# paultsw/wavenet-speech

Hardware: AMD Instinct MI355X
Metric: samples/sec fwd+bwd, 256-ch 30-block WaveNet @16k seq (higher is better)
Workload: dtype f32; 1 GPU; BASELINE.json configs[2]: WaveNet 256 ch, 30 blocks (3 x dilation 1..512), k=2, seq_len 16000, batch 16 per GPU, f32, full step (fwd+bwd+grad all-reduce+Adam); channels=256, blocks=30, seq_len=16000, batch_per_gpu=16, global_batch=16, parallelism=dp1, params=16037632, input=dense one-hot, init=reference

## Files before the change

wavenet_speech_amd/csrc/wn_api.hip:

```cpp
#include <hip/hip_runtime.h>

#include <algorithm>
#include <cstdio>
#include <cstdlib>
#include <cstdint>
#include <cstring>
#include <mutex>
#include <string>
#include <vector>

#include "../../include/wavenet_amd.h"
#include "wn_kernels.h"

using namespace wn;

#ifdef WN_STAMPS
namespace wn { extern int g_debug_kc; }
#endif

namespace {

thread_local std::string g_hip_err;

int hip_fail(hipError_t e, const char* what) {
// ... 204 lines not shown
    for (int i = 0; i < g.nslab; ++i) {
        a.slab_woff[i] = g.slab_woff[i];
        a.slab_nseg[i] = g.slab_nseg[i];
        a.slab_boff[i] = g.slab_boff[i];
    }
    a.wpacked = reinterpret_cast<float*>((char*)packed + off);
    a.bias = reinterpret_cast<float*>((char*)packed + off + align256((size_t)g.wfloats * 4));
    a.total = g.wfloats;
}

void fill_gemm_common(GemmArgs& a, const GemmPlan& g, const void* packed, size_t off, int first_slab, int nslab,
                      int B, int L, int ld, int halo) {
    std::memset(&a, 0, sizeof(a));
    a.wpacked = plan_w(packed, off);
    a.bias = plan_b(packed, off, g);
    a.nslab = nslab;
    for (int i = 0; i < nslab; ++i) {
        GemmSlab& s = a.slab[i];
        s.woff = g.slab_woff[first_slab + i];
        s.nseg = g.slab_nseg[first_slab + i];
        s.dst = g.slab_dst[first_slab + i];
        s.row0 = g.slab_row0[first_slab + i];
        s.boff = g.slab_boff[first_slab + i];
    }
    a.B = B; a.L = L; a.ld = ld; a.halo = halo;
    a.tiles_per_row = cdiv(L, kColTile);
    a.ncol = B * a.tiles_per_row;
}

inline void set_seg(GemmArgs& a, int i, const float* base, int c, int off, int nkb) {
    a.seg[i].base = base; a.seg[i].cp = cp8(c); a.seg[i].off = off; a.seg[i].nkb = nkb;
}

inline PackSrc mk_src(const float* p, int rows, int cols, int sr, int sc) {
    PackSrc s; s.ptr = p; s.rows = rows; s.cols = cols; s.stride_r = sr; s.stride_c = sc; return s;
}

struct WgradPlan {
    int WT = 1, npair = 0, ntile_total = 0, nsplit = 1;
    int Mp[kMaxPair], Np[kMaxPair], mt[kMaxPair], nt[kMaxPair], tile0[kMaxPair], rs_off[kMaxPair];
    long long slab_off[kMaxPair];
    long long slab_floats = 0;
    int rs_floats = 0;
    void add(int M, int N) {
        const int T = 64 * WT, i = npair++;
        mt[i] = cdiv(M, T); nt[i] = cdiv(N, T);
        Mp[i] = mt[i] * T; Np[i] = nt[i] * T;
        tile0[i] = ntile_total; ntile_total += mt[i] * nt[i];
        slab_off[i] = slab_floats; slab_floats += (long long)Mp[i] * Np[i];
        rs_off[i] = rs_floats; rs_floats += Mp[i];
    }
    void finish(int nchunk) {
        nsplit = std::max(1, 512 / std::max(1, ntile_total));
        nsplit = std::min(nsplit, std::max(1, nchunk));
        if (nsplit >= 16) nsplit = nsplit / 8 * 8;
    }
    bool xcd_map() const { return nsplit % 8 == 0; }
    size_t bytes() const { return (size_t)nsplit * (size_t)(slab_floats + rs_floats) * 4; }
};
inline int pick_wt(int maxdim) { return maxdim > 128 ? 4 : (maxdim > 64 ? 2 : 1); }

}


int wn_version(void) { return WN_VERSION; }

// ... 19 lines not shown
}

int wn_tap_offsets(int k, int d, int causal, int* off) {
    if (!off) return WN_ERR_NULL;
    if (k < 1 || d < 1) return WN_ERR_BAD_SHAPE;
    return tap_offsets(k, d, causal, off);
}

int wn_series_layout(int length, int max_abs_offset, int* ld, int* halo) {
    if (!ld || !halo) return WN_ERR_NULL;
    if (length <= 0 || max_abs_offset < 0) return WN_ERR_BAD_SHAPE;
    *halo = rup(max_abs_offset, 4);
    *ld = 2 * (*halo) + rup(length, kColTile);
    return WN_OK;
}

size_t wn_series_floats(int batch, int channels, int ld) { return (size_t)batch * cp8(channels) * (size_t)ld; }

size_t wn_block_packed_bytes(const wn_block_shape* s) {
    int off[WN_MAX_TAPS];
    if (check_block(s, off) != WN_OK) return 0;
    return plan_block(s).total;
}

int wn_block_pack(const wn_block_shape* s, const wn_block_params* p, void* packed, wn_stream_t stream) {
    int off[WN_MAX_TAPS];
    int rc = check_block(s, off);
    if (rc != WN_OK) return rc;
    if (!p || !packed || !p->w_tanh || !p->w_sigmoid || !p->w_res || !p->w_skip || !p->w_proj) return WN_ERR_NULL;
    hipStream_t st = (hipStream_t)stream;
    const BlockPlan bp = plan_block(s);
    const int Ci = s->in_channels, Co = s->out_channels, Ms = s->skip_rows, k = s->kernel_width;
    ProfScope prof(KC_PACK, 0.0, st);
    PackArgs a;
    {
        const GemmPlan& g = bp.fa;
        fill_pack_common(a, g, packed, bp.off_fa);
        for (int j = 0; j < k; ++j) {
            a.set[0].seg[j] = mk_src(p->w_tanh + j, Co, Ci, Ci * k, k);
            a.set[1].seg[j] = mk_src(p->w_sigmoid + j, Co, Ci, Ci * k, k);
        }
        a.set[0].bias0 = p->b_tanh; a.set[0].bias_rows = Co;
        a.set[1].bias0 = p->b_sigmoid; a.set[1].bias_rows = Co;
        const int pairs = tiles32(Co);
        for (int sl = 0; sl < g.nslab; ++sl)
            for (int m = 0; m < g.MT; ++m) {
                const int pair = sl * (g.MT / 2) + m / 2;
                a.tile[sl * g.MT + m].set = m & 1;
                a.tile[sl * g.MT + m].row0 = pair < pairs ? 32 * pair : -1;
            }
        WN_HIP(launch_pack(a, st), "pack(gate)");
    }
    {
        const GemmPlan& g = bp.fb;
        fill_pack_common(a, g, packed, bp.off_fb);
        a.set[0].seg[0] = mk_src(p->w_res, Co, Co, Co, 1);
        a.set[0].seg[1] = mk_src(p->w_proj, Co, Ci, Ci, 1);
        a.set[0].bias0 = p->b_res; a.set[0].bias1 = p->b_proj; a.set[0].bias_rows = Co;
        a.set[1].seg[0] = mk_src(p->w_skip, Ms, Co, Co, 1);
        a.set[1].bias0 = p->b_skip; a.set[1].bias_rows = Ms;
        for (int sl = 0; sl < g.nslab; ++sl)
            for (int m = 0; m < g.MT; ++m) {
                const bool skip = sl >= bp.fb_first_skip_slab;
                const int row0 = g.slab_row0[sl] + 32 * m;
                a.tile[sl * g.MT + m].set = skip ? 1 : 0;
                a.tile[sl * g.MT + m].row0 = row0 < (skip ? Ms : Co) ? row0 : -1;
            }
        WN_HIP(launch_pack(a, st), "pack(res+skip)");
    }
    {
        const GemmPlan& g = bp.ka;
        fill_pack_common(a, g, packed, bp.off_ka);
        a.set[0].seg[0] = mk_src(p->w_skip, Co, Ms, 1, Co);
        a.set[0].seg[1] = mk_src(p->w_res, Co, Co, 1, Co);
        for (int sl = 0; sl < g.nslab; ++sl)
            for (int m = 0; m < g.MT; ++m) {
                const int row0 = g.slab_row0[sl] + 32 * m;
                a.tile[sl * g.MT + m].set = 0;
                a.tile[sl * g.MT + m].row0 = row0 < Co ? row0 : -1;
            }
        WN_HIP(launch_pack(a, st), "pack(dz)");
    }
    {
        const GemmPlan& g = bp.kb;
        fill_pack_common(a, g, packed, bp.off_kb);
        for (int j = 0; j < k; ++j) {
            a.set[0].seg[2 * j] = mk_src(p->w_tanh + j, Ci, Co, k, Ci * k);
            a.set[0].seg[2 * j + 1] = mk_src(p->w_sigmoid + j, Ci, Co, k, Ci * k);
        }
        a.set[0].seg[2 * k] = mk_src(p->w_proj, Ci, Co, 1, Ci);
        for (int sl = 0; sl < g.nslab; ++sl)
            for (int m = 0; m < g.MT; ++m) {
                const int row0 = g.slab_row0[sl] + 32 * m;
                a.tile[sl * g.MT + m].set = 0;
                a.tile[sl * g.MT + m].row0 = row0 < Ci ? row0 : -1;
            }
        WN_HIP(launch_pack(a, st), "pack(dx)");
    }
    return WN_OK;
}

int wn_block_forward(const wn_block_shape* s, const void* packed, const float* x, float* r_out, float* skip,
                     int skip_accumulate, float* sg, float* z, wn_stream_t stream) {
    int off[WN_MAX_TAPS];
    int rc = check_block(s, off);
    if (rc != WN_OK) return rc;
    if (!packed || !x || !z) return WN_ERR_NULL;
    hipStream_t st = (hipStream_t)stream;
    const BlockPlan bp = plan_block(s);
    const int Ci = s->in_channels, Co = s->out_channels, Ms = s->skip_rows, k = s->kernel_width;
    const double BL = (double)s->batch * s->length;
    GemmArgs a;
    {
        const GemmPlan& g = bp.fa;
        fill_gemm_common(a, g, packed, bp.off_fa, 0, g.nslab, s->batch, s->length, s->ld, s->halo);
        for (int j = 0; j < k; ++j) set_seg(a, j, x, Ci, off[j], g.seg_nkb[j]);
        a.sg = sg; a.z = z; a.gate_cp = cp8(Co); a.gate_rows = Co;
        ProfScope prof(KC_GATE_GEMM, 2.0 * (2.0 * Co) * (double)(k * Ci) * BL, st);
        WN_HIP(launch_gemm(g.MT, EPI_GATE, a, st), "series_gemm<gate>");
    }
    {
        const GemmPlan& g = bp.fb;
        const double fl_r = 2.0 * Co * (double)(Co + Ci) * BL, fl_s = 2.0 * Ms * (double)Co * BL;
        if (r_out) {
            fill_gemm_common(a, g, packed, bp.off_fb, 0, bp.fb_first_skip_slab, s->batch, s->length, s->ld, s->halo);
            set_seg(a, 0, z, Co, 0, g.seg_nkb[0]);
            set_seg(a, 1, x, Ci, 0, g.seg_nkb[1]);
            a.dst[0].base = r_out; a.dst[0].cp = cp8(Co); a.dst[0].rows = Co; a.dst[0].accumulate = 0;
            ProfScope prof(KC_OUT_GEMM, fl_r, st);
            WN_HIP(launch_gemm(g.MT, EPI_LINEAR, a, st), "series_gemm<res>");
        }
// ... 67 lines not shown
    const int t = tiles32(s->skip_rows);
    g.MT = pick_mt(t);
    g.nseg = s->nblocks;
    for (int l = 0; l < s->nblocks; ++l) g.seg_nkb[l] = cp8(s->channels[l]) / 8;
    for (int i = 0; i < cdiv(t, g.MT); ++i) g.add_slab(s->nblocks, i * g.MT * 32, 0);
    return g;
}
}

size_t wn_skipsum_packed_bytes(const wn_skipsum_shape* s) {
    if (check_skipsum(s) != WN_OK) return 0;
    return plan_skipsum(s).bytes();
}

int wn_skipsum_pack(const wn_skipsum_shape* s, const float* const* w_skip, const float* bias_total, void* packed,
                    wn_stream_t stream) {
    int rc = check_skipsum(s);
    if (rc != WN_OK) return rc;
    if (!w_skip || !packed) return WN_ERR_NULL;
    for (int l = 0; l < s->nblocks; ++l) if (!w_skip[l]) return WN_ERR_NULL;
    hipStream_t st = (hipStream_t)stream;
    const GemmPlan g = plan_skipsum(s);
    ProfScope prof(KC_PACK, 0.0, st);
    PackArgs a;
    fill_pack_common(a, g, packed, 0);
    for (int l = 0; l < s->nblocks; ++l) a.set[0].seg[l] = mk_src(w_skip[l], s->skip_rows, s->channels[l], s->channels[l], 1);
    a.set[0].bias0 = bias_total; a.set[0].bias_rows = s->skip_rows;
    for (int sl = 0; sl < g.nslab; ++sl)
        for (int m = 0; m < g.MT; ++m) {
            const int row0 = g.slab_row0[sl] + 32 * m;
            a.tile[sl * g.MT + m].set = 0;
            a.tile[sl * g.MT + m].row0 = row0 < s->skip_rows ? row0 : -1;
        }
    WN_HIP(launch_pack(a, st), "pack(skipsum)");
    return WN_OK;
}

int wn_skipsum_forward(const wn_skipsum_shape* s, const void* packed, const float* const* z, float* skip, int accumulate,
                       wn_stream_t stream) {
    int rc = check_skipsum(s);
    if (rc != WN_OK) return rc;
    if (!packed || !z || !skip) return WN_ERR_NULL;
    for (int l = 0; l < s->nblocks; ++l) if (!z[l]) return WN_ERR_NULL;
    hipStream_t st = (hipStream_t)stream;
    const GemmPlan g = plan_skipsum(s);
    GemmArgs a;
    fill_gemm_common(a, g, packed, 0, 0, g.nslab, s->batch, s->length, s->ld, s->halo);
    double ksum = 0;
    for (int l = 0; l < s->nblocks; ++l) { set_seg(a, l, z[l], s->channels[l], 0, g.seg_nkb[l]); ksum += s->channels[l]; }
    a.dst[0].base = skip; a.dst[0].cp = cp8(s->skip_rows); a.dst[0].rows = s->skip_rows; a.dst[0].accumulate = accumulate ? 1 : 0;
    ProfScope prof(KC_SKIP_GEMM, 2.0 * s->skip_rows * ksum * (double)s->batch * s->length, st);
    WN_HIP(launch_gemm(g.MT, accumulate ? EPI_ACCUM : EPI_LINEAR, a, st), "series_gemm<skipsum>");
    return WN_OK;
}

namespace {
struct PairSpec { const float* A; int a_rows; const float* Bm; int b_rows; int off; int rowsum;
                  float* w; int sm, sn; float* b0; float* b1; };

int run_wgrad(const std::vector<PairSpec>& ps, int maxdim, int B, int L, int ld, int halo, void* workspace,
              size_t workspace_bytes, bool dry, size_t* need, int kc, hipStream_t st) {
    WgradPlan wp;
    wp.WT = pick_wt(maxdim);
    for (const PairSpec& p : ps) wp.add(p.a_rows, p.b_rows);
    const int cpr = cdiv(L, 32);
    wp.finish(B * cpr);
    if (need) *need = wp.bytes();
// ... 114 lines not shown
        GemmPlan& g = p.cf;
        const int t = tiles32(Co);
        g.MT = pick_mt(t); g.nseg = k;
        for (int j = 0; j < k; ++j) g.seg_nkb[j] = cp8(Ci) / 8;
        for (int i = 0; i < cdiv(t, g.MT); ++i) g.add_slab(k, i * g.MT * 32, 0);
    }
    {
        GemmPlan& g = p.cb;
        const int t = tiles32(Ci);
        g.MT = pick_mt(t); g.nseg = k;
        for (int j = 0; j < k; ++j) g.seg_nkb[j] = cp8(Co) / 8;
        for (int i = 0; i < cdiv(t, g.MT); ++i) g.add_slab(k, i * g.MT * 32, 0);
    }
    p.off_cf = 0; p.off_cb = p.cf.bytes(); p.total = p.off_cb + p.cb.bytes();
    return p;
}
}

size_t wn_conv_packed_bytes(const wn_conv_shape* s) {
    int off[WN_MAX_TAPS];
    if (check_conv(s, off) != WN_OK) return 0;
    return plan_conv(s).total;
}

int wn_conv_pack(const wn_conv_shape* s, const float* weight, const float* bias, void* packed, wn_stream_t stream) {
    int off[WN_MAX_TAPS];
    int rc = check_conv(s, off);
    if (rc != WN_OK) return rc;
    if (!weight || !packed) return WN_ERR_NULL;
    hipStream_t st = (hipStream_t)stream;
    const ConvPlan cp = plan_conv(s);
    const int Ci = s->in_channels, Co = s->out_channels, k = s->kernel_width;
    ProfScope prof(KC_PACK, 0.0, st);
    PackArgs a;
    {
        const GemmPlan& g = cp.cf;
        fill_pack_common(a, g, packed, cp.off_cf);
        for (int j = 0; j < k; ++j) a.set[0].seg[j] = mk_src(weight + j, Co, Ci, Ci * k, k);
        a.set[0].bias0 = bias; a.set[0].bias_rows = Co;
        for (int sl = 0; sl < g.nslab; ++sl)
            for (int m = 0; m < g.MT; ++m) {
                const int row0 = g.slab_row0[sl] + 32 * m;
                a.tile[sl * g.MT + m].set = 0;
                a.tile[sl * g.MT + m].row0 = row0 < Co ? row0 : -1;
            }
        WN_HIP(launch_pack(a, st), "pack(conv fwd)");
    }
    {
        const GemmPlan& g = cp.cb;
        fill_pack_common(a, g, packed, cp.off_cb);
        for (int j = 0; j < k; ++j) a.set[0].seg[j] = mk_src(weight + j, Ci, Co, k, Ci * k);
        for (int sl = 0; sl < g.nslab; ++sl)
            for (int m = 0; m < g.MT; ++m) {
                const int row0 = g.slab_row0[sl] + 32 * m;
                a.tile[sl * g.MT + m].set = 0;
                a.tile[sl * g.MT + m].row0 = row0 < Ci ? row0 : -1;
            }
        WN_HIP(launch_pack(a, st), "pack(conv bwd)");
    }
    return WN_OK;
}

int wn_conv_forward(const wn_conv_shape* s, const void* packed, const float* x, float* y, wn_stream_t stream) {
    int off[WN_MAX_TAPS];
    int rc = check_conv(s, off);
    if (rc != WN_OK) return rc;
    if (!packed || !x || !y) return WN_ERR_NULL;
    hipStream_t st = (hipStream_t)stream;
    const ConvPlan cp = plan_conv(s);
    const GemmPlan& g = cp.cf;
    GemmArgs a;
    fill_gemm_common(a, g, packed, cp.off_cf, 0, g.nslab, s->batch, s->length, s->ld, s->halo);
    for (int j = 0; j < s->kernel_width; ++j) set_seg(a, j, x, s->in_channels, off[j], g.seg_nkb[j]);
    a.dst[0].base = y; a.dst[0].cp = cp8(s->out_channels); a.dst[0].rows = s->out_channels; a.dst[0].accumulate = 0;
    ProfScope prof(KC_CONV_FWD, 2.0 * s->out_channels * (double)(s->kernel_width * s->in_channels) * s->batch * s->length, st);
    WN_HIP(launch_gemm(g.MT, EPI_LINEAR, a, st), "series_gemm<conv fwd>");
    return WN_OK;
}

int wn_conv_backward_data(const wn_conv_shape* s, const void* packed, const float* dy, float* dx, wn_stream_t stream) {
    int off[WN_MAX_TAPS];
    int rc = check_conv(s, off);
    if (rc != WN_OK) return rc;
    if (!packed || !dy || !dx) return WN_ERR_NULL;
    hipStream_t st = (hipStream_t)stream;
    const ConvPlan cp = plan_conv(s);
    const GemmPlan& g = cp.cb;
    GemmArgs a;
    fill_gemm_common(a, g, packed, cp.off_cb, 0, g.nslab, s->batch, s->length, s->ld, s->halo);
    a.bias = nullptr;
    for (int j = 0; j < s->kernel_width; ++j) set_seg(a, j, dy, s->out_channels, -off[j], g.seg_nkb[j]);
    a.dst[0].base = dx; a.dst[0].cp = cp8(s->in_channels); a.dst[0].rows = s->in_channels; a.dst[0].accumulate = 0;
// ... 98 lines not shown
```

wavenet_speech_amd/csrc/wn_gemm.hip:

```cpp
#include <cstdlib>

#include "wn_kernels.h"

namespace wn {

__device__ __forceinline__ int rowof(int r, int h) { return (r & 3) + 8 * (r >> 2) + 4 * h; }

__device__ __forceinline__ float sigmoid_f(float x) {
    const float e = __builtin_amdgcn_exp2f(-1.44269504088896341f * x);
    return __builtin_amdgcn_rcpf(1.0f + e);
}
__device__ __forceinline__ float tanh_f(float x) {
    const float ax = __builtin_fabsf(x);
    const float e = __builtin_amdgcn_exp2f(-2.88539008177792681f * ax);
    const float big = (1.0f - e) * __builtin_amdgcn_rcpf(1.0f + e);
    const float x2 = x * x;
    const float small = ax * (1.0f + x2 * (-0.333333333f + x2 * (0.133333333f + x2 * -0.0539682540f)));
    return __builtin_copysignf(ax < 0.125f ? small : big, x);
}

template <int NT> struct BVec;
template <> struct BVec<4> { typedef f32x4 reg_t; };
template <> struct BVec<2> { typedef float __attribute__((ext_vector_type(2))) reg_t; };

template <int MT, int NT, int EPI, int PFB, int WPS>
__global__ __launch_bounds__(64, WPS) void series_gemm_kernel(const GemmArgs a) {
    typedef typename BVec<NT>::reg_t breg_t;
    constexpr int COLS = 32 * NT;
    const int lane = threadIdx.x;
    const int n0 = lane & 31, h0 = lane >> 5;
#ifdef WN_STAMPS
    const unsigned long long st_t0 = __builtin_amdgcn_s_memtime(), st_r0 = __builtin_amdgcn_s_memrealtime();
    unsigned long long st_t1 = 0, st_t2 = 0;
#endif

    const int id = blockIdx.x;
    const int xcd = id & 7, local = id >> 3;
    const int slab_i = local % a.nslab;
    const int coltile = (local / a.nslab) * 8 + xcd;
    if (coltile >= a.ncol) return;
    const int b = coltile / a.tiles_per_row;
    const int t0 = (coltile - b * a.tiles_per_row) * COLS;
    const GemmSlab sl = a.slab[slab_i];
    const int ld = a.ld;

    f32x16 acc[MT][NT];
    const float* bias_p = (a.bias ? a.bias : a.wpacked) + sl.boff;
    const float bias_on = a.bias ? 1.0f : 0.0f;
#pragma unroll
    for (int m = 0; m < MT; ++m) {
#pragma unroll
        for (int r = 0; r < 16; ++r) {
            const float bv = bias_p[32 * m + rowof(r, h0)] * bias_on;
#pragma unroll
            for (int t = 0; t < NT; ++t) acc[m][t][r] = bv;
        }
    }

    int nkb = 0;
    for (int s = 0; s < sl.nseg; ++s) nkb += a.seg[s].nkb;

    constexpr unsigned kRsrcFlags = 0x00020000u;
    auto resource = [&](const float* base) {
        return __builtin_amdgcn_make_buffer_rsrc(const_cast<float*>(base), 0, 0xffffffffu, kRsrcFlags);
    };
    const __amdgpu_buffer_rsrc_t wrs = resource(a.wpacked + sl.woff);
    const unsigned a_off = lane * 16u;
    unsigned a_soff = 0;
    const long tilebase = (long)a.halo + t0;
    unsigned b_off[4];
#pragma unroll
    for (int q = 0; q < 4; ++q) b_off[q] = 4u * ((unsigned)(4 * h0 + q) * (unsigned)ld + (unsigned)(NT * n0));
    int seg = 0;
    int seg_left = a.seg[0].nkb;
    __amdgpu_buffer_rsrc_t brs = resource(a.seg[0].base + (long)b * a.seg[0].cp * ld);
    unsigned b_soff = 4u * (unsigned)(tilebase + a.seg[0].off);
    int b_left = nkb;
    const unsigned a_last = (unsigned)(nkb > 0 ? nkb - 1 : 0) * (MT * 1024u);

    f32x4 A[2][MT];
    breg_t B[4][4];
// ... 36 lines not shown
    for (int p = 0; p < PFB; ++p) loadB(B[p]);
#ifdef WN_STAMPS
    __builtin_amdgcn_sched_barrier(0);
    st_t1 = __builtin_amdgcn_s_memtime();
    __builtin_amdgcn_sched_barrier(0);
#endif
    int g0 = 0;
    for (; g0 + 4 <= nkb; g0 += 4) {
#pragma unroll
        for (int j = 0; j < 4; ++j) {
            loadA(A[(j + 1) & 1]);
            loadB(B[(j + PFB) & 3]);
            __builtin_amdgcn_sched_barrier(0);
            compute(A[j & 1], B[j & 3]);
            __builtin_amdgcn_sched_barrier(0);
        }
    }
#pragma unroll
    for (int j = 0; j < 3; ++j) {
        if (g0 + j < nkb) {
            loadA(A[(j + 1) & 1]);
            loadB(B[(j + PFB) & 3]);
            __builtin_amdgcn_sched_barrier(0);
            compute(A[j & 1], B[j & 3]);
            __builtin_amdgcn_sched_barrier(0);
        }
    }

#ifdef WN_STAMPS
    __builtin_amdgcn_sched_barrier(0);
    st_t2 = __builtin_amdgcn_s_memtime();
    __builtin_amdgcn_sched_barrier(0);
    struct StampOut {
        unsigned long long* p; unsigned long long t0, r0, t1, t2; int lane;
        __device__ ~StampOut() {
            __builtin_amdgcn_sched_barrier(0);
            const unsigned long long t_issued = __builtin_amdgcn_s_memtime();
            __builtin_amdgcn_sched_barrier(0);
            asm volatile("s_waitcnt vmcnt(0)" ::: "memory");
            if (p && lane == 0) {
                p[0] = t0; p[1] = t1; p[2] = t2; p[3] = __builtin_amdgcn_s_memtime();
                p[4] = r0; p[5] = __builtin_amdgcn_s_memrealtime();
                p[6] = __builtin_amdgcn_s_getreg(63492);
                p[7] = (unsigned long long)__builtin_amdgcn_s_getreg(63508) | ((t_issued - t2) << 32);
            }
        }
    } stamp_out{a.stamps ? a.stamps + 8ull * blockIdx.x : nullptr, st_t0, st_r0, st_t1, st_t2, lane};
#endif
    const int lane_e = (int)__builtin_amdgcn_mbcnt_hi(~0u, __builtin_amdgcn_mbcnt_lo(~0u, 0u));
    const int n = lane_e & 31, h = lane_e >> 5;
    const long colbase = tilebase + NT * n;
    const int c0 = t0 + NT * n;
    if (c0 >= a.L) return;
    auto clip = [&](breg_t v) {
#pragma unroll
        for (int t = 1; t < NT; ++t)
            if (c0 + t >= a.L) v[t] = 0.0f;
        return v;
    };

    if constexpr (EPI == EPI_LINEAR) {
        const GemmDst d = a.dst[sl.dst];
#pragma unroll
        for (int m = 0; m < MT; ++m) {
#pragma unroll
            for (int r = 0; r < 16; ++r) {
                const int row = sl.row0 + 32 * m + rowof(r, h);
                if (row < d.rows) {
                    float* p = d.base + ((long)b * d.cp + row) * ld + colbase;
                    breg_t v;
#pragma unroll
                    for (int t = 0; t < NT; ++t) v[t] = acc[m][t][r];
                    *reinterpret_cast<breg_t*>(p) = clip(v);
                }
            }
            __builtin_amdgcn_sched_barrier(0);
        }
    } else if constexpr (EPI == EPI_ACCUM) {
        const GemmDst d = a.dst[sl.dst];
        constexpr int RB = 8, BPT = 16 / RB, NBATCH = MT * BPT;
        breg_t old[2][RB];
        float* const tile = d.base + (long)b * d.cp * ld + colbase;
        auto fetch = [&](int bi, breg_t (&dst)[RB]) {
            const int m = bi / BPT, r0 = (bi % BPT) * RB;
#pragma unroll
            for (int i = 0; i < RB; ++i) {
                int row = sl.row0 + 32 * m + rowof(r0 + i, h);
                row = row < d.rows ? row : d.rows - 1;
                dst[i] = *reinterpret_cast<const breg_t*>(tile + (long)row * ld);
            }
        };
        fetch(0, old[0]);
#pragma unroll
        for (int bi = 0; bi < NBATCH; ++bi) {
            if (bi + 1 < NBATCH) fetch(bi + 1, old[(bi + 1) & 1]);
            __builtin_amdgcn_sched_barrier(0);
            const int m = bi / BPT, r0 = (bi % BPT) * RB;
#pragma unroll
            for (int i = 0; i < RB; ++i) {
                const int row = sl.row0 + 32 * m + rowof(r0 + i, h);
                if (row < d.rows) {
                    breg_t v;
#pragma unroll
                    for (int t = 0; t < NT; ++t) v[t] = acc[m][t][r0 + i] + old[bi & 1][i][t];
                    *reinterpret_cast<breg_t*>(tile + (long)row * ld) = clip(v);
                }
            }
            __builtin_amdgcn_sched_barrier(0);
        }
    } else if constexpr (EPI == EPI_GATE) {
#pragma unroll
        for (int i = 0; i < MT / 2; ++i) {
#pragma unroll
            for (int r = 0; r < 16; ++r) {
                const int ch = sl.row0 + 32 * i + rowof(r, h);
                if (ch < a.gate_rows) {
                    breg_t vs, vz;
#pragma unroll
                    for (int t = 0; t < NT; ++t) {
                        const float tt = tanh_f(acc[2 * i][t][r]);
                        const float ss = sigmoid_f(acc[2 * i + 1][t][r]);
                        vs[t] = ss;
                        vz[t] = tt * ss;
                    }
                    const long o = ((long)b * a.gate_cp + ch) * ld + colbase;
                    *reinterpret_cast<breg_t*>(a.z + o) = clip(vz);
                    if (a.sg) *reinterpret_cast<breg_t*>(a.sg + o) = clip(vs);
                }
            }
            __builtin_amdgcn_sched_barrier(0);
        }
    } else {
        constexpr int RB = (MT == 4) ? 8 : 4;
        constexpr int BPT = 16 / RB;
        constexpr int NBATCH = MT * BPT;
        breg_t vt[2][RB], vs[2][RB];
        auto fetch = [&](int bi, breg_t (&ft)[RB], breg_t (&fs)[RB]) {
            const int m = bi / BPT, r0 = (bi % BPT) * RB;
#pragma unroll
            for (int i = 0; i < RB; ++i) {
                int ch = sl.row0 + 32 * m + rowof(r0 + i, h);
                ch = ch < a.gate_rows ? ch : a.gate_rows - 1;
                const long o = ((long)b * a.gate_cp + ch) * ld + colbase;
                ft[i] = *reinterpret_cast<const breg_t*>(a.z + o);
                fs[i] = *reinterpret_cast<const breg_t*>(a.sg + o);
            }
        };
        fetch(0, vt[0], vs[0]);
#pragma unroll
        for (int bi = 0; bi < NBATCH; ++bi) {
            if (bi + 1 < NBATCH) fetch(bi + 1, vt[(bi + 1) & 1], vs[(bi + 1) & 1]);
            __builtin_amdgcn_sched_barrier(0);
            const int m = bi / BPT, r0 = (bi % BPT) * RB;
#pragma unroll
            for (int i = 0; i < RB; ++i) {
                const int r = r0 + i;
                const int ch = sl.row0 + 32 * m + rowof(r, h);
                if (ch < a.gate_rows) {
                    const long o = ((long)b * a.gate_cp + ch) * ld + colbase;
                    const breg_t z_ = vt[bi & 1][i], sg_ = vs[bi & 1][i];
                    breg_t va, vg;
#pragma unroll
                    for (int t = 0; t < NT; ++t) {
                        const float dz = acc[m][t][r];
                        const float tt = sg_[t] > 0.0f ? z_[t] / sg_[t] : 0.0f;
                        va[t] = dz * (sg_[t] - z_[t] * tt);
                        vg[t] = dz * z_[t] * (1.0f - sg_[t]);
                    }
                    *reinterpret_cast<breg_t*>(a.da + o) = clip(va);
                    *reinterpret_cast<breg_t*>(a.dg + o) = clip(vg);
                }
            }
            __builtin_amdgcn_sched_barrier(0);
        }
    }
}

#ifdef WN_STAMPS
static unsigned long long* g_stamp_buf = nullptr;
static int g_stamp_kc = -1;
int g_debug_kc = -1;
extern "C" void wn_debug_set_stamp_buffer(void* p) { g_stamp_buf = (unsigned long long*)p; }
extern "C" void wn_debug_set_stamp_class(int kc) { g_stamp_kc = kc; }
extern "C" unsigned wn_debug_last_grid = 0;
#endif

template <int MT, int NT, int EPI, int PFB, int WPS>
static hipError_t launch_one(GemmArgs a, hipStream_t st) {
#ifdef WN_STAMPS
    const bool stamp_this = g_stamp_buf && (g_stamp_kc < 0 || g_stamp_kc == g_debug_kc);
    a.stamps = stamp_this ? g_stamp_buf : nullptr;
#endif
    a.tiles_per_row = (a.L + 32 * NT - 1) / (32 * NT);
    a.ncol = a.B * a.tiles_per_row;
    const int ncol8 = (a.ncol + 7) / 8 * 8;
    const unsigned grid = (unsigned)(a.nslab * ncol8);
#ifdef WN_STAMPS
    if (stamp_this) wn_debug_last_grid = grid;
#endif
    hipLaunchKernelGGL((series_gemm_kernel<MT, NT, EPI, PFB, WPS>), dim3(grid), dim3(64), 0, st, a);
    return hipGetLastError();
}

static int gemm_variant() {
    static int v = -1;
    if (v < 0) {
        const char* e = getenv("WN_GEMM_VARIANT");
        v = e ? atoi(e) : 0;
    }
    return v;
}

template <int EPI>
static hipError_t launch_epi(int MT, const GemmArgs& a, hipStream_t st) {
    const int v = gemm_variant();
    if (MT == 4) {
        if (v == 1) return launch_one<4, 4, EPI, 1, 1>(a, st);
        return launch_one<4, 4, EPI, 3, 1>(a, st);
    }
    if (MT == 2) return launch_one<2, 4, EPI, 3, 2>(a, st);
    if constexpr (EPI != EPI_GATE) {
        if (MT == 1) return launch_one<1, 4, EPI, 3, 2>(a, st);
    }
    return hipErrorInvalidValue;
}

hipError_t launch_gemm(int MT, int epi, const GemmArgs& a, hipStream_t st) {
    if (a.nslab <= 0 || a.B <= 0 || a.L <= 0) return hipSuccess;
    switch (epi) {
        case EPI_LINEAR: return launch_epi<EPI_LINEAR>(MT, a, st);
        case EPI_GATE: return launch_epi<EPI_GATE>(MT, a, st);
// ... 8 lines not shown
```

wavenet_speech_amd/csrc/wn_kernels.h:

```cpp
#pragma once
#include <hip/hip_runtime.h>
#include <stdint.h>

namespace wn {

typedef float f32x16 __attribute__((ext_vector_type(16)));
typedef float f32x4 __attribute__((ext_vector_type(4)));

constexpr int kMaxSeg = 32;
constexpr int kMaxSlab = 32;
constexpr int kMaxDst = 2;
constexpr int kColTile = 128;

struct GemmSeg {
    const float* base;
    int cp;
    int off;
    int nkb;
    int _pad;
};

struct GemmSlab {
    long long woff;
    int nseg;
// ... 27 lines not shown
    int tiles_per_row;
    int ncol;
    unsigned long long* stamps;
};

enum { EPI_LINEAR = 0, EPI_GATE = 1, EPI_DGATE = 2, EPI_ACCUM = 3 };

struct PackSrc {
    const float* ptr;
    int rows, cols;
    int stride_r, stride_c;
};
struct PackSet {
    PackSrc seg[kMaxSeg];
    const float* bias0;
    const float* bias1;
    int bias_rows;
    int _pad;
};
struct PackTile { int set; int row0; };
struct PackArgs {
    PackSet set[2];
    PackTile tile[kMaxSlab * 4];
    int seg_nkb[kMaxSeg];
    long long slab_woff[kMaxSlab];
    int slab_nseg[kMaxSlab];
    int slab_boff[kMaxSlab];
    int nslab, MT;
    float* wpacked;
    float* bias;
    long long total;
};

constexpr int kMaxPair = 2 * 8 + 3;
constexpr int kMaxReduceDst = 56;
struct WgradPair {
    const float* A; const float* Bm;
    int a_cp, b_cp;
    int off;
    int mt, nt;
    int tile0;
    long long slab_off;
    int Mp, Np;
    int rowsum;
    int rs_off;
};
struct WgradArgs {
    WgradPair pair[kMaxPair];
    int npair;
    int ntile_total;
    int nsplit;
    int B, L, ld, halo;
    int chunks_per_row;
    int nchunk;
    float* slab;
    float* rowsum;
    long long slab_floats;
    int rs_floats;
    int xcd_map;
};

struct ReduceDst {
    float* w;
    int M, N, sm, sn;
    long long slab_off; int Np;
    float* b0; float* b1;
    int rs_off;
    float post;
};
struct ReduceArgs {
    ReduceDst d[kMaxReduceDst];
    int npair, nsplit;
    const float* slab; const float* rowsum;
    long long slab_floats; int rs_floats;
    const float* dyn_inv;
};

static_assert(sizeof(ReduceArgs) <= 4096 && sizeof(WgradArgs) <= 4096, "kernel arguments are limited to 4 KiB");

hipError_t launch_gemm(int MT, int epi, const GemmArgs& a, hipStream_t st);
hipError_t launch_pack(const PackArgs& a, hipStream_t st);
hipError_t launch_wgrad(int WT, const WgradArgs& a, hipStream_t st);
hipError_t launch_wgrad_reduce(const ReduceArgs& a, hipStream_t st);
hipError_t launch_nll_forward(const float* logits, const long long* target, float* lse, float* partial, int* bad_targets, int B,
                              int C, int L, hipStream_t st);
hipError_t launch_nll_backward(const float* logits, const long long* target, const float* lse, const float* gscale,
                               float* dlogits, int B, int C, int L, hipStream_t st);

}
```

wavenet_speech_amd/csrc/wn_pack.hip:

```cpp
#include "wn_kernels.h"

namespace wn {

__global__ __launch_bounds__(256) void pack_kernel(const PackArgs a) {
    const long long idx = (long long)blockIdx.x * 256 + threadIdx.x;
    if (idx < a.total) {
        int slab = 0;
        while (slab + 1 < a.nslab && idx >= a.slab_woff[slab + 1]) ++slab;
        const long long rel = idx - a.slab_woff[slab];
        const int q = (int)(rel & 3);
        const int lane = (int)((rel >> 2) & 63);
        const long long gm = rel >> 8;
        const int m = (int)(gm % a.MT);
        int g = (int)(gm / a.MT);
        int s = 0;
        while (g >= a.seg_nkb[s]) { g -= a.seg_nkb[s]; ++s; }
        const int c = 8 * g + 4 * (lane >> 5) + q;
        const PackTile t = a.tile[slab * a.MT + m];
        float v = 0.0f;
        if (t.row0 >= 0) {
            const PackSrc src = a.set[t.set].seg[s];
            const int r = t.row0 + (lane & 31);
            if (src.ptr && r < src.rows && c < src.cols) v = src.ptr[(long long)r * src.stride_r + (long long)c * src.stride_c];
        }
        a.wpacked[idx] = v;
    }
    const long long nb = (long long)a.nslab * a.MT * 32;
    if (idx < nb && a.bias) {
        const int slab = (int)(idx / (a.MT * 32));
        const int rr = (int)(idx % (a.MT * 32));
        const PackTile t = a.tile[slab * a.MT + rr / 32];
        float v = 0.0f;
        if (t.row0 >= 0) {
            const PackSet& ps = a.set[t.set];
            const int r = t.row0 + (rr & 31);
            if (r < ps.bias_rows) {
                if (ps.bias0) v += ps.bias0[r];
                if (ps.bias1) v += ps.bias1[r];
            }
        }
        a.bias[a.slab_boff[slab] + rr] = v;
    }
}

hipError_t launch_pack(const PackArgs& a, hipStream_t st) {
    long long n = a.total;
    const long long nb = (long long)a.nslab * a.MT * 32;
    if (nb > n) n = nb;
    if (n <= 0) return hipSuccess;
    hipLaunchKernelGGL(pack_kernel, dim3((unsigned)((n + 255) / 256)), dim3(256), 0, st, a);
    return hipGetLastError();
}

}
```

Baseline: 96.67 samples/s.

## Batch weight-pack launches and make series GEMM a persistent grid-stride kernel

Several per-block pack kernel launches are merged into one launch that carries a small job table, which cuts launch count. The series GEMM kernel becomes persistent: the grid is capped at a resident count derived from the CU count, and each workgroup loops over tiles. The gate-backward epilogue now uses buffer loads and stores with 32-bit offsets and a deeper prefetch for MT=2. The linear epilogue drops 64-bit address math. The bias asm trick and the slab_boff replacement in pack change addressing, and the bias offset now assumes contiguous slabs.

Result: no change. 97.32 samples/s (median of 6 runs) (+0.7%).

```diff
diff --git a/wavenet_speech_amd/csrc/wn_api.hip b/wavenet_speech_amd/csrc/wn_api.hip
--- a/wavenet_speech_amd/csrc/wn_api.hip
+++ b/wavenet_speech_amd/csrc/wn_api.hip
@@ -260,6 +260,23 @@
     a.seg[i].base = base; a.seg[i].cp = cp8(c); a.seg[i].off = off; a.seg[i].nkb = nkb;
 }
 
+struct PackBatch {
+    PackJobs t;
+    hipStream_t st;
+    explicit PackBatch(hipStream_t s) : st(s) { std::memset(&t, 0, sizeof(t)); }
+    hipError_t flush() {
+        const hipError_t e = launch_pack(t, st);
+        std::memset(&t, 0, sizeof(t));
+        return e;
+    }
+    hipError_t add(const PackArgs& a) {
+        if (pack_jobs_add(t, a)) return hipSuccess;
+        const hipError_t e = flush();
+        if (e != hipSuccess) return e;
+        return pack_jobs_add(t, a) ? hipSuccess : hipErrorInvalidValue;
+    }
+};
+
 inline PackSrc mk_src(const float* p, int rows, int cols, int sr, int sc) {
     PackSrc s; s.ptr = p; s.rows = rows; s.cols = cols; s.stride_r = sr; s.stride_c = sc; return s;
 }
@@ -345,6 +362,7 @@
     const BlockPlan bp = plan_block(s);
     const int Ci = s->in_channels, Co = s->out_channels, Ms = s->skip_rows, k = s->kernel_width;
     ProfScope prof(KC_PACK, 0.0, st);
+    PackBatch batch(st);
     PackArgs a;
     {
         const GemmPlan& g = bp.fa;
@@ -362,7 +380,7 @@
                 a.tile[sl * g.MT + m].set = m & 1;
                 a.tile[sl * g.MT + m].row0 = pair < pairs ? 32 * pair : -1;
             }
-        WN_HIP(launch_pack(a, st), "pack(gate)");
+        WN_HIP(batch.add(a), "pack(gate)");
     }
     {
         const GemmPlan& g = bp.fb;
@@ -379,7 +397,7 @@
                 a.tile[sl * g.MT + m].set = skip ? 1 : 0;
                 a.tile[sl * g.MT + m].row0 = row0 < (skip ? Ms : Co) ? row0 : -1;
             }
-        WN_HIP(launch_pack(a, st), "pack(res+skip)");
+        WN_HIP(batch.add(a), "pack(res+skip)");
     }
     {
         const GemmPlan& g = bp.ka;
@@ -392,7 +410,7 @@
                 a.tile[sl * g.MT + m].set = 0;
                 a.tile[sl * g.MT + m].row0 = row0 < Co ? row0 : -1;
             }
-        WN_HIP(launch_pack(a, st), "pack(dz)");
+        WN_HIP(batch.add(a), "pack(dz)");
     }
     {
         const GemmPlan& g = bp.kb;
@@ -408,8 +426,9 @@
                 a.tile[sl * g.MT + m].set = 0;
                 a.tile[sl * g.MT + m].row0 = row0 < Ci ? row0 : -1;
             }
-        WN_HIP(launch_pack(a, st), "pack(dx)");
-    }
+        WN_HIP(batch.add(a), "pack(dx)");
+    }
+    WN_HIP(batch.flush(), "pack(block)");
     return WN_OK;
 }
 
@@ -543,7 +562,9 @@
             a.tile[sl * g.MT + m].set = 0;
             a.tile[sl * g.MT + m].row0 = row0 < s->skip_rows ? row0 : -1;
         }
-    WN_HIP(launch_pack(a, st), "pack(skipsum)");
+    PackBatch batch(st);
+    WN_HIP(batch.add(a), "pack(skipsum)");
+    WN_HIP(batch.flush(), "pack(skipsum)");
     return WN_OK;
 }
 
@@ -724,6 +745,7 @@
     const ConvPlan cp = plan_conv(s);
     const int Ci = s->in_channels, Co = s->out_channels, k = s->kernel_width;
     ProfScope prof(KC_PACK, 0.0, st);
+    PackBatch batch(st);
     PackArgs a;
     {
         const GemmPlan& g = cp.cf;
@@ -736,7 +758,7 @@
                 a.tile[sl * g.MT + m].set = 0;
                 a.tile[sl * g.MT + m].row0 = row0 < Co ? row0 : -1;
             }
-        WN_HIP(launch_pack(a, st), "pack(conv fwd)");
+        WN_HIP(batch.add(a), "pack(conv fwd)");
     }
     {
         const GemmPlan& g = cp.cb;
@@ -748,8 +770,9 @@
                 a.tile[sl * g.MT + m].set = 0;
                 a.tile[sl * g.MT + m].row0 = row0 < Ci ? row0 : -1;
             }
-        WN_HIP(launch_pack(a, st), "pack(conv bwd)");
-    }
+        WN_HIP(batch.add(a), "pack(conv bwd)");
+    }
+    WN_HIP(batch.flush(), "pack(conv)");
     return WN_OK;
 }
 
diff --git a/wavenet_speech_amd/csrc/wn_gemm.hip b/wavenet_speech_amd/csrc/wn_gemm.hip
--- a/wavenet_speech_amd/csrc/wn_gemm.hip
+++ b/wavenet_speech_amd/csrc/wn_gemm.hip
@@ -1,3 +1,4 @@
+#include <atomic>
 #include <cstdlib>
 
 #include "wn_kernels.h"
@@ -24,21 +25,23 @@
 template <> struct BVec<2> { typedef float __attribute__((ext_vector_type(2))) reg_t; };
 
 template <int MT, int NT, int EPI, int PFB, int WPS>
-__global__ __launch_bounds__(64, WPS) void series_gemm_kernel(const GemmArgs a) {
+__device__ __forceinline__ void series_gemm_tile(const GemmArgs& a, const int local, const int xcd, const int st_seq) {
     typedef typename BVec<NT>::reg_t breg_t;
     constexpr int COLS = 32 * NT;
-    const int lane = threadIdx.x;
-    const int n0 = lane & 31, h0 = lane >> 5;
+    auto lane_id = [] {
+        int l;
+        asm volatile("v_mbcnt_lo_u32_b32 %0, -1, 0\n\tv_mbcnt_hi_u32_b32 %0, -1, %0" : "=v"(l));
+        return l;
+    };
 #ifdef WN_STAMPS
     const unsigned long long st_t0 = __builtin_amdgcn_s_memtime(), st_r0 = __builtin_amdgcn_s_memrealtime();
     unsigned long long st_t1 = 0, st_t2 = 0;
 #endif
-
-    const int id = blockIdx.x;
-    const int xcd = id & 7, local = id >> 3;
     const int slab_i = local % a.nslab;
     const int coltile = (local / a.nslab) * 8 + xcd;
     if (coltile >= a.ncol) return;
+    const int lane = lane_id();
+    const int n0 = lane & 31, h0 = lane >> 5;
     const int b = coltile / a.tiles_per_row;
     const int t0 = (coltile - b * a.tiles_per_row) * COLS;
     const GemmSlab sl = a.slab[slab_i];
@@ -46,7 +49,9 @@
 
     f32x16 acc[MT][NT];
     const float* bias_p = (a.bias ? a.bias : a.wpacked) + sl.boff;
-    const float bias_on = a.bias ? 1.0f : 0.0f;
+    unsigned bias_bits = a.bias ? 0x3f800000u : 0u;
+    asm volatile("" : "+s"(bias_bits));
+    const float bias_on = __builtin_bit_cast(float, bias_bits);
 #pragma unroll
     for (int m = 0; m < MT; ++m) {
 #pragma unroll
@@ -149,7 +154,7 @@
     st_t2 = __builtin_amdgcn_s_memtime();
     __builtin_amdgcn_sched_barrier(0);
     struct StampOut {
-        unsigned long long* p; unsigned long long t0, r0, t1, t2; int lane;
+        unsigned long long* p; unsigned long long t0, r0, t1, t2; int lane, seq;
         __device__ ~StampOut() {
             __builtin_amdgcn_sched_barrier(0);
             const unsigned long long t_issued = __builtin_amdgcn_s_memtime();
@@ -158,13 +163,13 @@
             if (p && lane == 0) {
                 p[0] = t0; p[1] = t1; p[2] = t2; p[3] = __builtin_amdgcn_s_memtime();
                 p[4] = r0; p[5] = __builtin_amdgcn_s_memrealtime();
-                p[6] = __builtin_amdgcn_s_getreg(63492);
+                p[6] = (unsigned long long)__builtin_amdgcn_s_getreg(63492) | ((unsigned long long)seq << 32);
                 p[7] = (unsigned long long)__builtin_amdgcn_s_getreg(63508) | ((t_issued - t2) << 32);
             }
         }
-    } stamp_out{a.stamps ? a.stamps + 8ull * blockIdx.x : nullptr, st_t0, st_r0, st_t1, st_t2, lane};
-#endif
-    const int lane_e = (int)__builtin_amdgcn_mbcnt_hi(~0u, __builtin_amdgcn_mbcnt_lo(~0u, 0u));
+    } stamp_out{a.stamps ? a.stamps + 8ull * (unsigned)(local * 8 + xcd) : nullptr, st_t0, st_r0, st_t1, st_t2, lane, st_seq};
+#endif
+    const int lane_e = lane_id();
     const int n = lane_e & 31, h = lane_e >> 5;
     const long colbase = tilebase + NT * n;
     const int c0 = t0 + NT * n;
@@ -178,13 +183,14 @@
 
     if constexpr (EPI == EPI_LINEAR) {
         const GemmDst d = a.dst[sl.dst];
+        float* const tile = d.base + ((long)b * d.cp * ld + tilebase);
 #pragma unroll
         for (int m = 0; m < MT; ++m) {
 #pragma unroll
             for (int r = 0; r < 16; ++r) {
                 const int row = sl.row0 + 32 * m + rowof(r, h);
                 if (row < d.rows) {
-                    float* p = d.base + ((long)b * d.cp + row) * ld + colbase;
+                    float* p = tile + ((unsigned)row * (unsigned)ld + (unsigned)(NT * n));
                     breg_t v;
 #pragma unroll
                     for (int t = 0; t < NT; ++t) v[t] = acc[m][t][r];
@@ -251,22 +257,39 @@
         constexpr int RB = (MT == 4) ? 8 : 4;
         constexpr int BPT = 16 / RB;
         constexpr int NBATCH = MT * BPT;
-        breg_t vt[2][RB], vs[2][RB];
+        constexpr int AHEAD = (MT == 2) ? 2 : 1;
+        constexpr int NS = AHEAD + 1;
+        breg_t vt[NS][RB], vs[NS][RB];
+        const long plane = (long)b * a.gate_cp * ld + tilebase;
+        const __amdgpu_buffer_rsrc_t zrs = resource(a.z + plane), srs = resource(a.sg + plane);
+        const __amdgpu_buffer_rsrc_t dars = resource(a.da + plane), dgrs = resource(a.dg + plane);
+        const unsigned o_first = 4u * ((unsigned)(sl.row0 + 4 * h) * (unsigned)ld + (unsigned)(NT * n));
+        const unsigned o_last = 4u * ((unsigned)(a.gate_rows - 1) * (unsigned)ld + (unsigned)(NT * n));
+        const unsigned rowbytes = 4u * (unsigned)ld;
+        auto rowoff = [&](int m, int r) { return min(o_first + (unsigned)(32 * m + rowof(r, 0)) * rowbytes, o_last); };
+        auto ld_row = [&](__amdgpu_buffer_rsrc_t rs, unsigned o) {
+            if constexpr (NT == 4) return __builtin_bit_cast(breg_t, __builtin_amdgcn_raw_buffer_load_b128(rs, o, 0, 0));
+            else return __builtin_bit_cast(breg_t, __builtin_amdgcn_raw_buffer_load_b64(rs, o, 0, 0));
+        };
+        auto st_row = [&](__amdgpu_buffer_rsrc_t rs, unsigned o, breg_t v) {
+            if constexpr (NT == 4) __builtin_amdgcn_raw_buffer_store_b128(__builtin_bit_cast(__attribute__((__vector_size__(4 * sizeof(unsigned)))) unsigned, v), rs, o, 0, 0);
+            else __builtin_amdgcn_raw_buffer_store_b64(__builtin_bit_cast(__attribute__((__vector_size__(2 * sizeof(unsigned)))) unsigned, v), rs, o, 0, 0);
+        };
         auto fetch = [&](int bi, breg_t (&ft)[RB], breg_t (&fs)[RB]) {
             const int m = bi / BPT, r0 = (bi % BPT) * RB;
 #pragma unroll
             for (int i = 0; i < RB; ++i) {
-                int ch = sl.row0 + 32 * m + rowof(r0 + i, h);
-                ch = ch < a.gate_rows ? ch : a.gate_rows - 1;
-                const long o = ((long)b * a.gate_cp + ch) * ld + colbase;
-                ft[i] = *reinterpret_cast<const breg_t*>(a.z + o);
-                fs[i] = *reinterpret_cast<const breg_t*>(a.sg + o);
+                const unsigned o = rowoff(m, r0 + i);
+                ft[i] = ld_row(zrs, o);
+                fs[i] = ld_row(srs, o);
             }
         };
-        fetch(0, vt[0], vs[0]);
+#pragma unroll
+        for (int p = 0; p < AHEAD; ++p)
+            if (p < NBATCH) fetch(p, vt[p], vs[p]);
 #pragma unroll
         for (int bi = 0; bi < NBATCH; ++bi) {
-            if (bi + 1 < NBATCH) fetch(bi + 1, vt[(bi + 1) & 1], vs[(bi + 1) & 1]);
+            if (bi + AHEAD < NBATCH) fetch(bi + AHEAD, vt[(bi + AHEAD) % NS], vs[(bi + AHEAD) % NS]);
             __builtin_amdgcn_sched_barrier(0);
             const int m = bi / BPT, r0 = (bi % BPT) * RB;
 #pragma unroll
@@ -274,8 +297,8 @@
                 const int r = r0 + i;
                 const int ch = sl.row0 + 32 * m + rowof(r, h);
                 if (ch < a.gate_rows) {
-                    const long o = ((long)b * a.gate_cp + ch) * ld + colbase;
-                    const breg_t z_ = vt[bi & 1][i], sg_ = vs[bi & 1][i];
+                    const unsigned o = rowoff(m, r);
+                    const breg_t z_ = vt[bi % NS][i], sg_ = vs[bi % NS][i];
                     breg_t va, vg;
 #pragma unroll
                     for (int t = 0; t < NT; ++t) {
@@ -284,13 +307,22 @@
                         va[t] = dz * (sg_[t] - z_[t] * tt);
                         vg[t] = dz * z_[t] * (1.0f - sg_[t]);
                     }
-                    *reinterpret_cast<breg_t*>(a.da + o) = clip(va);
-                    *reinterpret_cast<breg_t*>(a.dg + o) = clip(vg);
+                    st_row(dars, o, clip(va));
+                    st_row(dgrs, o, clip(vg));
                 }
             }
             __builtin_amdgcn_sched_barrier(0);
         }
     }
+}
+
+template <int MT, int NT, int EPI, int PFB, int WPS>
+__global__ __launch_bounds__(64, WPS) void series_gemm_kernel(const GemmArgs a) {
+    const int xcd = blockIdx.x & 7;
+    const int nlocal = a.nslab * ((a.ncol + 7) >> 3);
+    const int lstride = (int)(gridDim.x >> 3);
+    int seq = 0;
+    for (int local = blockIdx.x >> 3; local < nlocal; local += lstride) series_gemm_tile<MT, NT, EPI, PFB, WPS>(a, local, xcd, seq++);
 }
 
 #ifdef WN_STAMPS
@@ -302,6 +334,19 @@
 extern "C" unsigned wn_debug_last_grid = 0;
 #endif
 
+static int device_cus() {
+    constexpr int kMaxDev = 64;
+    static std::atomic<int> cus[kMaxDev];
+    int dev = 0;
+    if (hipGetDevice(&dev) != hipSuccess || dev < 0 || dev >= kMaxDev) dev = 0;
+    int n = cus[dev].load(std::memory_order_relaxed);
+    if (n <= 0) {
+        if (hipDeviceGetAttribute(&n, hipDeviceAttributeMultiprocessorCount, dev) != hipSuccess || n <= 0) n = 8;
+        cus[dev].store(n, std::memory_order_relaxed);
+    }
+    return n;
+}
+
 template <int MT, int NT, int EPI, int PFB, int WPS>
 static hipError_t launch_one(GemmArgs a, hipStream_t st) {
 #ifdef WN_STAMPS
@@ -311,9 +356,11 @@
     a.tiles_per_row = (a.L + 32 * NT - 1) / (32 * NT);
     a.ncol = a.B * a.tiles_per_row;
     const int ncol8 = (a.ncol + 7) / 8 * 8;
-    const unsigned grid = (unsigned)(a.nslab * ncol8);
-#ifdef WN_STAMPS
-    if (stamp_this) wn_debug_last_grid = grid;
+    const unsigned ntiles = (unsigned)(a.nslab * ncol8);
+    const unsigned resident = (unsigned)device_cus() * 4u * WPS / 8u * 8u;
+    const unsigned grid = ntiles < resident ? ntiles : resident;
+#ifdef WN_STAMPS
+    if (stamp_this) wn_debug_last_grid = ntiles;
 #endif
     hipLaunchKernelGGL((series_gemm_kernel<MT, NT, EPI, PFB, WPS>), dim3(grid), dim3(64), 0, st, a);
     return hipGetLastError();
diff --git a/wavenet_speech_amd/csrc/wn_kernels.h b/wavenet_speech_amd/csrc/wn_kernels.h
--- a/wavenet_speech_amd/csrc/wn_kernels.h
+++ b/wavenet_speech_amd/csrc/wn_kernels.h
@@ -83,6 +83,32 @@
     long long total;
 };
 
+constexpr int kPackJobs = 4;
+constexpr int kPackSrcs = 40;
+constexpr int kPackSlabs = 96;
+constexpr int kPackTiles = 256;
+struct PackJob {
+    float* wpacked;
+    float* bias;
+    long long total;
+    const float* bias0[2];
+    const float* bias1[2];
+    int bias_rows[2];
+    int src0[2], nsrc[2];
+    int nslab, MT;
+    int slab0, tile0;
+    int block0, nblocks;
+    int seg_nkb[kMaxSeg];
+};
+struct PackJobs {
+    PackJob job[kPackJobs];
+    PackSrc src[kPackSrcs];
+    long long slab_woff[kPackSlabs];
+    int tile[kPackTiles];
+    int njob, nsrc, nslab, ntile;
+};
+static_assert(sizeof(PackJobs) <= 4096, "PackJobs travels as a kernel argument");
+
 constexpr int kMaxPair = 2 * 8 + 3;
 constexpr int kMaxReduceDst = 56;
 struct WgradPair {
@@ -130,7 +156,8 @@
 static_assert(sizeof(ReduceArgs) <= 4096 && sizeof(WgradArgs) <= 4096, "kernel arguments are limited to 4 KiB");
 
 hipError_t launch_gemm(int MT, int epi, const GemmArgs& a, hipStream_t st);
-hipError_t launch_pack(const PackArgs& a, hipStream_t st);
+bool pack_jobs_add(PackJobs& t, const PackArgs& a);
+hipError_t launch_pack(const PackJobs& t, hipStream_t st);
 hipError_t launch_wgrad(int WT, const WgradArgs& a, hipStream_t st);
 hipError_t launch_wgrad_reduce(const ReduceArgs& a, hipStream_t st);
 hipError_t launch_nll_forward(const float* logits, const long long* target, float* lse, float* partial, int* bad_targets, int B,
diff --git a/wavenet_speech_amd/csrc/wn_pack.hip b/wavenet_speech_amd/csrc/wn_pack.hip
--- a/wavenet_speech_amd/csrc/wn_pack.hip
+++ b/wavenet_speech_amd/csrc/wn_pack.hip
@@ -1,13 +1,19 @@
+#include <cstring>
+
 #include "wn_kernels.h"
 
 namespace wn {
 
-__global__ __launch_bounds__(256) void pack_kernel(const PackArgs a) {
-    const long long idx = (long long)blockIdx.x * 256 + threadIdx.x;
+__global__ __launch_bounds__(256) void pack_kernel(const PackJobs t) {
+    int j = 0;
+    while (j + 1 < t.njob && (int)blockIdx.x >= t.job[j + 1].block0) ++j;
+    const PackJob& a = t.job[j];
+    const long long idx = (long long)((int)blockIdx.x - a.block0) * 256 + threadIdx.x;
     if (idx < a.total) {
+        const long long* slab_woff = t.slab_woff + a.slab0;
         int slab = 0;
-        while (slab + 1 < a.nslab && idx >= a.slab_woff[slab + 1]) ++slab;
-        const long long rel = idx - a.slab_woff[slab];
+        while (slab + 1 < a.nslab && idx >= slab_woff[slab + 1]) ++slab;
+        const long long rel = idx - slab_woff[slab];
         const int q = (int)(rel & 3);
         const int lane = (int)((rel >> 2) & 63);
         const long long gm = rel >> 8;
@@ -16,11 +22,11 @@
         int s = 0;
         while (g >= a.seg_nkb[s]) { g -= a.seg_nkb[s]; ++s; }
         const int c = 8 * g + 4 * (lane >> 5) + q;
-        const PackTile t = a.tile[slab * a.MT + m];
+        const int tl = t.tile[a.tile0 + slab * a.MT + m];
         float v = 0.0f;
-        if (t.row0 >= 0) {
-            const PackSrc src = a.set[t.set].seg[s];
-            const int r = t.row0 + (lane & 31);
+        if (tl >= 0 && s < a.nsrc[tl & 1]) {
+            const PackSrc src = t.src[a.src0[tl & 1] + s];
+            const int r = (tl >> 1) + (lane & 31);
             if (src.ptr && r < src.rows && c < src.cols) v = src.ptr[(long long)r * src.stride_r + (long long)c * src.stride_c];
         }
         a.wpacked[idx] = v;
@@ -29,26 +35,58 @@
     if (idx < nb && a.bias) {
         const int slab = (int)(idx / (a.MT * 32));
         const int rr = (int)(idx % (a.MT * 32));
-        const PackTile t = a.tile[slab * a.MT + rr / 32];
+        const int tl = t.tile[a.tile0 + slab * a.MT + rr / 32];
         float v = 0.0f;
-        if (t.row0 >= 0) {
-            const PackSet& ps = a.set[t.set];
-            const int r = t.row0 + (rr & 31);
-            if (r < ps.bias_rows) {
-                if (ps.bias0) v += ps.bias0[r];
-                if (ps.bias1) v += ps.bias1[r];
+        if (tl >= 0) {
+            const int set = tl & 1;
+            const int r = (tl >> 1) + (rr & 31);
+            if (r < a.bias_rows[set]) {
+                if (a.bias0[set]) v += a.bias0[set][r];
+                if (a.bias1[set]) v += a.bias1[set][r];
             }
         }
-        a.bias[a.slab_boff[slab] + rr] = v;
+        a.bias[(long long)slab * a.MT * 32 + rr] = v;
     }
 }
 
-hipError_t launch_pack(const PackArgs& a, hipStream_t st) {
+bool pack_jobs_add(PackJobs& t, const PackArgs& a) {
+    int nsrc[2];
+    for (int i = 0; i < 2; ++i) {
+        nsrc[i] = 0;
+        for (int s = 0; s < kMaxSeg; ++s)
+            if (a.set[i].seg[s].ptr) nsrc[i] = s + 1;
+    }
+    const int ntile = a.nslab * a.MT;
+    if (t.njob >= kPackJobs || t.nsrc + nsrc[0] + nsrc[1] > kPackSrcs || t.nslab + a.nslab > kPackSlabs || t.ntile + ntile > kPackTiles)
+        return false;
+    PackJob& j = t.job[t.njob];
+    std::memset(&j, 0, sizeof(j));
+    j.wpacked = a.wpacked; j.bias = a.bias; j.total = a.total;
+    j.nslab = a.nslab; j.MT = a.MT;
+    for (int i = 0; i < 2; ++i) {
+        j.bias0[i] = a.set[i].bias0; j.bias1[i] = a.set[i].bias1; j.bias_rows[i] = a.set[i].bias_rows;
+        j.src0[i] = t.nsrc; j.nsrc[i] = nsrc[i];
+        for (int s = 0; s < nsrc[i]; ++s) t.src[t.nsrc++] = a.set[i].seg[s];
+    }
+    for (int s = 0; s < kMaxSeg; ++s) j.seg_nkb[s] = a.seg_nkb[s];
+    j.slab0 = t.nslab;
+    for (int s = 0; s < a.nslab; ++s) t.slab_woff[t.nslab++] = a.slab_woff[s];
+    j.tile0 = t.ntile;
+    for (int i = 0; i < ntile; ++i) t.tile[t.ntile++] = a.tile[i].row0 < 0 ? -1 : ((a.tile[i].row0 << 1) | (a.tile[i].set & 1));
     long long n = a.total;
     const long long nb = (long long)a.nslab * a.MT * 32;
     if (nb > n) n = nb;
-    if (n <= 0) return hipSuccess;
-    hipLaunchKernelGGL(pack_kernel, dim3((unsigned)((n + 255) / 256)), dim3(256), 0, st, a);
+    j.block0 = t.njob ? t.job[t.njob - 1].block0 + t.job[t.njob - 1].nblocks : 0;
+    j.nblocks = (int)((n + 255) / 256);
+    ++t.njob;
+    return true;
+}
+
+hipError_t launch_pack(const PackJobs& t, hipStream_t st) {
+    if (t.njob <= 0) return hipSuccess;
+    const int nblocks = t.job[t.njob - 1].block0 + t.job[t.njob - 1].nblocks;
+    if (nblocks <= 0) return hipSuccess;
+    hipLaunchKernelGGL(pack_kernel, dim3((unsigned)nblocks), dim3(256), 0, st, t);
     return hipGetLastError();
 }
 
```
